# cve-mohd/flow-sim

Measured on AMD Instinct MI355X. Metric: reach-timesteps/sec (batched Preissmann Newton step), higher is better.
Workload: dtype f64

## Files before the change

flow-sim_amd/csrc/fs_abi.hip:

```cpp
#include <hip/hip_runtime.h>

#include <algorithm>
#include <cmath>
#include <condition_variable>
#include <cstdio>
#include <cstdlib>
#include <cstring>
#include <functional>
#include <limits>
#include <mutex>
#include <string>
#include <thread>
#include <vector>

#include "fs_buffer.hpp"
#include "fs_entries.hpp"
#include "fs_host_pack.hpp"

#include <rocprofiler-sdk-roctx/roctx.h>
namespace {
struct TraceRange {
  explicit TraceRange(const char *name) { roctxRangePushA(name); }
  ~TraceRange() { roctxRangePop(); }
};
// ... 163 lines not shown
  fs::DeviceBuffer iters, status;
  fs::DeviceBuffer it_done;
  fs::DeviceBuffer ends_dev;
  fs::PinnedBuffer ends_pin;
  fs::DeviceBuffer open_dev;
  fs::PinnedBuffer open_pin;
  fs::DeviceBuffer derived[8];
  fs::DeviceBuffer dbg;
  Staging stage;
  fs::DeviceBuffer kc_scratch;
  int passes = 0;
  fs::DeviceBuffer team_mail;
  fs::DeviceBuffer team_sync;
  int team_size = 0;
  uint32_t team_epoch = 0;
};

namespace {

template <typename F> auto with_real(const fs_batch *b, F &&f) { return b->d.dtype == FS_F64 ? f(double()) : f(float()); }

dim3 grid_256(size_t n) { return dim3((unsigned)((n + 255) / 256)); }

int upload_to(fs_batch *b, void *dst, const double *src, size_t n) {
  TraceRange range_("flowsim:upload");
  const bool f64 = b->esz == sizeof(double);
  if (f64 || n * b->esz < kStageMin || b->stage.init() != 0) {
    if (f64) {
      HIP_TRY(hipMemcpyAsync(dst, src, n * sizeof(double), hipMemcpyHostToDevice, b->stream));
      HIP_TRY(hipStreamSynchronize(b->stream));
// ... 120 lines not shown
  a.geo_reach_stride = (int64_t)b->geo_reach_stride; a.poly_reach_stride = (int64_t)b->poly_reach_stride;
  a.reach_nodes = b->reach_nodes.get<int32_t>(); a.reach_scheme = b->reach_scheme.get<R>();
  a.reach_kinds = (b->kinds_per_reach[0] || b->kinds_per_reach[1]) ? b->reach_kinds.get<int32_t>() : nullptr;
  fs::BCDesc<R> *bc[2] = {&a.us, &a.ds};
  for (int s = 0; s < 2; ++s) {
    bc[s]->kind = b->bc_kind[s]; bc[s]->stride = b->bc_stride[s];
    bc[s]->params = b->bc_params[s].get<R>(); bc[s]->target = b->bc_target[s].get<R>(); bc[s]->tgt = R(0);
  }
  a.Yprev = b->Yprev.get<R>(); a.stage_hist = b->stage_hist.get<R>(); a.trace = b->trace.get<R>(); a.hydro = b->hydro.get<R>();
  a.iters = b->iters.get<int32_t>(); a.status = b->status.get<int32_t>();
  a.hist_h = b->hist_h.get<R>(); a.hist_Q = b->hist_Q.get<R>();
  a.dbg = b->dbg.get<unsigned long long>();
  a.kc_scratch = b->kc_scratch.get<R>(); a.passes = b->passes;
  a.team_size = b->team_size; a.team_mail = b->team_mail.get<R>(); a.team_sync = b->team_sync.get<unsigned long long>(); a.team_epoch = b->team_epoch;
  a.iter_budget = 0; a.it_done = b->it_done.get<int32_t>();
}

int launch_steps(fs_batch *b, int n_steps, int iter_budget) {
  TraceRange range_(iter_budget > 0 ? "flowsim:iterate" : "flowsim:step");
  std::string why;
  const int hetero = (b->reach_nodes ? 1 : 0) | ((b->reach_scheme || b->kinds_per_reach[0] || b->kinds_per_reach[1]) ? 2 : 0);
  fs::Query q;
  q.dtype = b->d.dtype; q.sec = b->d.section_mode; q.N = b->d.n_nodes; q.usk = b->bc_kind[0]; q.dsk = b->bc_kind[1];
  q.need_diag = (b->d.flags & (FS_FLAG_HISTORY | FS_FLAG_TRACE | FS_FLAG_MONITOR)) != 0; q.need_any = iter_budget > 0; q.hetero = hetero;
  const int chosen = fs::pick(kEntries, kNumEntries, q, fs::overrides_from_environment(), &why);
  const Entry *k = chosen < 0 ? nullptr : &kEntries[chosen];
  if (!k && why.rfind("FS_KERNEL_INDEX", 0) == 0) return fail("fs_batch_step: " + why);
  if (!k && (b->bc_kind[0] == FS_BC_STORAGE_CURVE || b->bc_kind[1] == FS_BC_STORAGE_CURVE))
    return fail("fs_batch_step: FS_BC_STORAGE_CURVE needs section mode FS_SEC_TABLE or FS_SEC_IRREGULAR");
  if (!k) return fail("fs_batch_step: no kernel instantiation for this boundary kind at this size");
  b->kern = k;
  b->passes = 0;
  if (k->key.longk) {
    const size_t chunk = (size_t)64 * k->key.W * k->key.M;
    b->passes = (int)((b->d.n_nodes + chunk - 1) / chunk);
    const bool recompute = b->d.section_mode == FS_SEC_RECT_UNIFORM || b->d.section_mode == FS_SEC_TRAP_UNIFORM;
    const size_t need = recompute ? 0 : (size_t)b->d.n_reaches * 4 * b->passes * chunk;
    HIP_TRY(b->kc_scratch.reserve(need * b->esz));
  }
  b->team_size = 0;
  if (k->key.team) {
    const size_t chunk = (size_t)64 * k->key.W * k->key.M, B = b->d.n_reaches;
    b->team_size = (int)((b->d.n_nodes + chunk - 1) / chunk);
    const size_t need = B * 2 * ((size_t)b->team_size * k->key.W + 1) * fs::kTeamWords * 2;
    bool grew = false;
    HIP_TRY(b->team_mail.reserve(need * sizeof(double), &grew));
    if (grew) HIP_TRY(hipMemsetAsync(b->team_mail.get(), 0, need * sizeof(double), b->stream));
    ++b->team_epoch;
    HIP_TRY(b->team_sync.ensure(sizeof(unsigned long long)));
    HIP_TRY(hipMemsetAsync(b->team_sync.get(), 0, sizeof(unsigned long long), b->stream));
  }
  HIP_TRY(hipEventRecord(b->ev0, b->stream));
  with_real(b, [&](auto real) {
    fs::KernelArgs<decltype(real)> a; fill_args(b, n_steps, a);
    a.iter_budget = iter_budget;
    b->kern->fn(&a, b->d.n_reaches, b->stream);
  });
  HIP_TRY(hipGetLastError());
  HIP_TRY(hipEventRecord(b->ev1, b->stream));
  b->timed = true; b->launches = 1;
  return 0;
}


int check_side(const char *entry, int32_t side) {
  if (side != FS_UPSTREAM && side != FS_DOWNSTREAM) return fail(std::string(entry) + ": side must be FS_UPSTREAM or FS_DOWNSTREAM");
// ... 32 lines not shown

int fill_side_kinds(fs_batch *b, int side, int kind) {
  const size_t B = b->d.n_reaches;
  const std::vector<int32_t> same(B, kind);
  HIP_TRY(hipMemcpy(b->reach_kinds.get<int32_t>() + (size_t)side * B, same.data(), B * 4, hipMemcpyHostToDevice));
  return 0;
}

int begin_at_level0(fs_batch *b) {
  const size_t B = b->d.n_reaches, L = b->d.max_levels;
  HIP_TRY(hipMemsetAsync(b->status.get(), 0, B * 4, b->stream));
  HIP_TRY(hipMemsetAsync(b->iters.get(), 0, L * B * 4, b->stream));
  HIP_TRY(hipMemsetAsync(b->Yprev.get(), 0, B * b->esz, b->stream));
  if (b->trace) HIP_TRY(hipMemsetAsync(b->trace.get(), 0, L * FS_TRACE_CAP * B * b->esz, b->stream));
  HIP_TRY(hipMemsetAsync(b->it_done.get(), 0, B * 4, b->stream));
  b->level = 0; b->iterating = false; b->restart_level = 0;
  b->have_state = true;
  return 0;
}

int init_batch(fs_batch *b) {
  HIP_TRY(hipSetDevice(b->d.device));
  HIP_TRY(hipStreamCreateWithFlags(&b->stream, hipStreamNonBlocking));
  HIP_TRY(hipEventCreate(&b->ev0));
  HIP_TRY(hipEventCreate(&b->ev1));
  const size_t B = b->d.n_reaches, N = b->d.n_nodes, L = b->d.max_levels, esz = b->esz;
  auto zeroed = [&](fs::DeviceBuffer &buf, size_t bytes) -> int {
    HIP_TRY(buf.ensure(bytes));
    HIP_TRY(hipMemsetAsync(buf.get(), 0, bytes, b->stream));
    return 0;
  };
  for (fs::DeviceBuffer *p : {&b->hk, &b->Qk, &b->hg, &b->Qg}) HIP_TRY(p->ensure(B * N * esz));
  if (zeroed(b->hydro, L * 4 * B * esz) || zeroed(b->iters, L * B * 4) || zeroed(b->status, B * 4) || zeroed(b->Yprev, B * esz) ||
      zeroed(b->stage_hist, L * B * esz) || zeroed(b->it_done, B * 4)) return -1;
  if ((b->d.flags & FS_FLAG_TRACE) && zeroed(b->trace, L * FS_TRACE_CAP * B * esz)) return -1;
  if (b->d.flags & FS_FLAG_HISTORY) {
    HIP_TRY(b->hist_h.ensure(L * B * N * esz));
    HIP_TRY(b->hist_Q.ensure(L * B * N * esz));
  }
#ifdef FS_STAMP
  if (zeroed(b->dbg, B * 16 * 12 * 8)) return -1;
#endif
  HIP_TRY(hipStreamSynchronize(b->stream));
  if (B * N * esz >= kStageMin) (void)b->stage.init();
  return 0;
}

}

extern "C" {

int fs_abi_version(void) { return FS_ABI_VERSION; }

int fs_device_count(void) {
  int n = 0;
  if (hipGetDeviceCount(&n) != hipSuccess) return 0;
// ... 546 lines not shown

double fs_batch_last_step_ms(fs_batch *b) {
  if (!b || !b->timed) return -1.0;
  float ms = 0.f;
  if (hipEventSynchronize(b->ev1) != hipSuccess) return -1.0;
  if (hipEventElapsedTime(&ms, b->ev0, b->ev1) != hipSuccess) return -1.0;
  return (double)ms;
}

int32_t fs_batch_last_launch_count(fs_batch *b) { return b ? b->launches : 0; }

#ifdef FS_STAMP
int fs_debug_stamps(fs_batch *b, unsigned long long *out) {
  if (!b || !out || !b->dbg) return fail("fs_debug_stamps: not available");
  HIP_TRY(hipStreamSynchronize(b->stream));
  HIP_TRY(hipMemcpy(out, b->dbg.get(), (size_t)b->d.n_reaches * 16 * 12 * 8, hipMemcpyDeviceToHost));
  return 0;
}
#endif

int32_t fs_kernel_table_size(void) { return kNumEntries; }

int fs_kernel_table_entry(int32_t i, int32_t *out) {
  if (i < 0 || i >= kNumEntries || !out) return fail("fs_kernel_table_entry: index out of range");
  const fs::KernelKey &e = kEntries[i].key;
  out[0] = e.dtype; out[1] = e.sec; out[2] = e.M; out[3] = e.W; out[4] = e.full; out[5] = e.bck; out[6] = e.diag; out[7] = e.longk;
  return 0;
}

int32_t fs_batch_kernel_index(fs_batch *b) { return (b && b->kern) ? (int32_t)(b->kern - kEntries) : -1; }

int32_t fs_kernel_table_entry_tail(int32_t i) { return (i >= 0 && i < kNumEntries) ? kEntries[i].key.tail : -2; }
int32_t fs_kernel_table_entry_team(int32_t i) { return (i >= 0 && i < kNumEntries) ? kEntries[i].key.team : -2; }

int32_t fs_batch_poly_tables(fs_batch *b) { return (b && b->poly_x) ? (b->poly_K > 0 ? 1 : 0) : -1; }

int fs_batch_kernel_info(fs_batch *b, int32_t *cells_per_thread, int32_t *waves_per_reach, int32_t *lds_bytes,
                         int32_t *vgprs) {
  if (!b) return fail("null handle");
  hipFuncAttributes at;
  HIP_TRY(hipFuncGetAttributes(&at, b->kern->kp));
  if (cells_per_thread) *cells_per_thread = b->kern->key.M;
  if (waves_per_reach) *waves_per_reach = b->kern->key.W;
  if (lds_bytes) *lds_bytes = (int32_t)at.sharedSizeBytes;
  if (vgprs) *vgprs = at.numRegs;
// ... 5 lines not shown
```

flow-sim_amd/csrc/fs_dispatch.hpp:

```cpp
#pragma once
#include <algorithm>
#include <cstdio>
#include <cstdlib>
#include <string>
#include <tuple>

#include "../../include/flowsim_abi.h"
#include "fs_entry_list.hpp"

#ifndef FS_ST_HD
#ifdef __HIPCC__
#define FS_ST_HD __host__ __device__
#else
#define FS_ST_HD
#endif
#endif

namespace fs {

FS_ST_HD constexpr bool bc_is_light(int kind) { return kind != FS_BC_RATING_POWER && kind < FS_BC_STORAGE_CURVE; }

struct KernelKey {
  int dtype;
  int sec;
  int M;
  int W;
  int full;
  int bck;
  int diag;
  int longk;
  int tail;
  int team;
};
#define FS_KEY(KIND, R, DT, SEC, M, W, FULL, BCK, DIAG, TAIL) \
  fs::KernelKey{DT, SEC, M, W, FULL, (int)(BCK), DIAG, FS_KIND_##KIND == FS_KIND_LONG, TAIL, FS_KIND_##KIND == FS_KIND_TEAM}
// ... 3 lines not shown
  int N;
  int usk, dsk;
  bool need_diag = false;
  bool need_any = false;
  int hetero = 0;
};

struct Overrides {
  bool force_index = false;
  int index = 0;
  std::string index_text;
  int M = 0, W = 0;
  bool general_only = false;
  bool no_team = false;
  int team_M = -1;
};

inline Overrides overrides_from_environment() {
  Overrides o;
  if (const char *env = std::getenv("FS_KERNEL_INDEX")) { o.force_index = true; o.index = std::atoi(env); o.index_text = env; }
  if (const char *env = std::getenv("FS_KERNEL_SHAPE")) std::sscanf(env, "%d,%d", &o.M, &o.W);
  if (const char *env = std::getenv("FS_KERNEL_GENERAL")) o.general_only = env[0] == '1';
  o.no_team = std::getenv("FS_NO_TEAM") != nullptr;
  if (const char *env = std::getenv("FS_TEAM_M")) o.team_M = std::max(std::atoi(env), 0);
  return o;
}

inline bool fits(const KernelKey &k, const Query &q, const Overrides &o) {
  if (k.dtype != q.dtype || k.sec != q.sec) return false;
  const long grid = 64L * k.W * k.M, cap = grid * ((k.longk || k.team) ? 64 / k.W : 1);
  if (q.N > cap || q.N > 32768) return false;
  if (k.full && (k.team ? q.N % grid != 0 : q.N != cap)) return false;
  if (k.tail >= 0 && (q.N - 1) % k.M != k.tail) return false;
  if (k.team && (q.N <= 4096 || q.N <= grid || o.no_team || (o.team_M >= 0 && o.team_M != k.M))) return false;
  if ((q.hetero & 1) && (k.full || k.tail >= 0)) return false;
  if ((q.hetero & 2) && k.bck > 0) return false;
  if (q.need_diag && !k.diag) return false;
  if (q.need_any && k.bck != -1) return false;
// ... 34 lines not shown
```

flow-sim_amd/csrc/fs_kernel.hpp:

```cpp
#pragma once
#include <type_traits>
#include "fs_device.hpp"
#include "fs_poly.hpp"

namespace fs {

#ifdef FS_STAMP
#define FS_T(i)                                                         \
  do {                                                                  \
    const unsigned long long now_ = __builtin_amdgcn_s_memtime();       \
    stamp_[i] += now_ - tprev_;                                         \
    tprev_ = now_;                                                      \
  } while (0)
#else
#define FS_T(i) do { } while (0)
#endif

template <typename R> __host__ __device__ constexpr R finite_max() { return sizeof(R) == 8 ? R(1.7976931348623157e308) : R(3.4028234e38); }
template <typename R> __host__ __device__ constexpr R eps_of() { return sizeof(R) == 8 ? R(2.220446049250313e-16) : R(1.1920929e-7); }

__device__ __forceinline__ int hi_abs(double v) { return __double2hiint(v) & 0x7fffffff; }
__device__ __forceinline__ int hi_abs(float v) { return __float_as_int(v) & 0x7fffffff; }
template <typename R> __host__ __device__ constexpr int growth_limit_bits() { return sizeof(R) == 8 ? ((1023 + 10) << 20) : ((127 + 10) << 23); }
__device__ __forceinline__ int max_(int a, int b) { return a > b ? a : b; }
// ... 21 lines not shown
  R *trace;
  unsigned long long *dbg;
  int64_t geo_reach_stride;
  int64_t poly_reach_stride;
  const int32_t *reach_nodes;
  const R *reach_scheme;
  const int32_t *reach_kinds;
  const R *poly_tz;
  int32_t poly_K;
  R *kc_scratch;
  int32_t passes;
  int32_t team_size;
  R *team_mail;
  unsigned long long *team_sync;
  uint32_t team_epoch;
};
constexpr int kTeamSlots = 64;
constexpr unsigned long long kTeamPatience = 16000000000ull;
constexpr int kTeamWords = 12;

template <typename R, int SEC> struct Geometry;

constexpr int kTeamSleep = 1;
typedef unsigned int fs_u4 __attribute__((ext_vector_type(4)));
constexpr int kTeamAuxSc1 = 16;
__device__ __forceinline__ void team_put2(__amdgpu_buffer_rsrc_t r, unsigned off, unsigned long long bits, unsigned long long tag) {
  fs_u4 v;
  v.x = (unsigned)bits; v.y = (unsigned)(bits >> 32); v.z = (unsigned)tag; v.w = (unsigned)(tag >> 32);
  __builtin_amdgcn_raw_buffer_store_b128(v, r, off, 0, kTeamAuxSc1);
}
// ... 16 lines not shown
    n = a.geo_uniform[(size_t)FS_RU_MANNING * a.B + reach];
    z_us = a.geo_uniform[(size_t)FS_RU_Z_US * a.B + reach];
    z_ds = a.geo_uniform[(size_t)FS_RU_Z_DS * a.B + reach];
    rb = R(1) / b; rn = R(1) / n;
    inv_nm1 = R(1) / R(n_nodes - 1);
    dz = (z_ds - z_us) * inv_nm1;
  }
  __device__ __forceinline__ R bed_step(int) const { return dz; }
  __device__ __forceinline__ R terms_T() const { return b; }
  __device__ __forceinline__ R rT_const() const { return rb; }
  __device__ __forceinline__ R bed(int node) const {
    const R w2 = R(node) * inv_nm1;
    return z_us * (R(1) - w2) + z_ds * w2;
  }
  __device__ __forceinline__ NodeTerms<R> terms(int, R h, R Q) const { return node_terms_rect(b, rb, n, h, Q); }
  __device__ __forceinline__ SecParams<R> section(int node) const {
    SecParams<R> s;
    s.z = bed(node); s.b = b; s.m = R(0); s.nm = n; s.nl = n; s.nr = n; s.hbf = R(0);
    s.bl = R(0); s.br = R(0); s.mfp = R(0); s.curv = R(0); s.compound = false;
    s.sm = R(1); s.rnm = rn; s.sfp = R(1); s.Tb = b; s.Am = R(0); s.Pm = b; s.km15 = s.kl15 = s.kr15 = R(0);
    return s;
  }
  template <int BCK, int SIDE>
  __device__ __forceinline__ BCRow<R> boundary(const BCDesc<R> &bc, int reach, int B, int level, int node, R h, R Q,
                                               R Qold, R dt, R Yprev, R *Ynew, int *flag) const {
    if (BCK == 1 || (BCK >= 2 && bc_is_light(BCK - 2)))
      return bc_eval_rect(pinned<BCK, SIDE>(bc), (LdsParams<R>)bc.params, level, b, n, node == 0 ? z_us : z_ds, h, Q, Qold, dt, Yprev, Ynew, flag);
    return bc_eval<BCK != 0>(pinned<BCK, SIDE>(bc), reach, B, level, section(node), h, Q, Qold, dt, Yprev, Ynew, flag);
  }
};
// ... 203 lines not shown
}

template <typename R, int SEC, int M, int W, bool RAGGED = true, int BCK = 0, bool DIAG = true, int TAIL = -1, bool TEAM = false>
__global__ __launch_bounds__(64 * W, (min_waves<R, SEC, M, W, BCK, TEAM>())) void preissmann_step_kernel(const KernelArgs<R> a) {
  static_assert(M >= 2, "a lane's segment needs two rows (its up and its down row)");
  constexpr bool kTail = TAIL >= 0;
  constexpr bool kTeam = TEAM;
  static_assert(!kTeam || (W > 1 && BCK >= 0 && !kTail), "team form: multi-wave kernels, boundary kinds of the device");
  static_assert(!kTail || (RAGGED && W == 1 && TAIL < M && SEC == FS_SEC_TABLE && BCK >= 2), "tail-only form: ragged one-wave table kernels compiled for a boundary pair");
  constexpr int T = 64 * W;
  using Geo = Geometry<R, SEC>;
  constexpr int kSaveTermsMaxMF64 = 2;
  constexpr bool kSaveTerms = !Geometry<R, SEC>::kConstT && (M <= 2 || (sizeof(R) == 8 && M <= kSaveTermsMaxMF64));
  constexpr bool kRegGeo = SEC == FS_SEC_TABLE && W == 1 && M <= 2;
  constexpr bool kFlatBC = BCK >= 2 && sizeof(R) == 8 && SEC == FS_SEC_TRAP_UNIFORM;
  __shared__ Smem<R, M, W, kSaveTerms, kTeam> sm;

  const int t = threadIdx.x, lane = t & 63, wave = t >> 6;
  int job = blockIdx.x;
  if constexpr (kTeam) {
    if (t == 0) sm.xjob = (int)__hip_atomic_fetch_add(a.team_sync, 1ull, __ATOMIC_RELAXED, __HIP_MEMORY_SCOPE_AGENT);
    __syncthreads();
    job = sm.xjob;
  }
  const int G = kTeam ? a.team_size : 1;
  const int reach = kTeam ? job / G : job, member = kTeam ? job - reach * G : 0;
  const int gt = member * T + t;
  auto mbox = [&](int par) __attribute__((always_inline)) {
    const size_t bytes = (size_t)(G * W + 1) * kTeamWords * 16;
    char *base = reinterpret_cast<char *>(a.team_mail) + ((size_t)reach * 2 + par) * bytes;
// ... 63 lines not shown
  auto last_node_terms = [&](const NodeTerms<R> &first) __attribute__((always_inline)) {
    auto rol = [](R v) { return dpp_mov<0x134>(v); };
    NodeTerms<R> r;
    r.A = rol(first.A); r.T = rol(first.T); r.Se = rol(first.Se); r.eAT = rol(first.eAT); r.eQ = rol(first.eQ); r.v = rol(first.v);
    r.rT = rol(first.rT);
    return r;
  };
  auto write_level_constants = [&](const R(&hh)[M + 1], const R(&QQ)[M + 1]) __attribute__((always_inline)) {
    NodeTerms<R> L = terms_at(0, hh[0], QQ[0]);
    NodeTerms<R> Rlast;
    if (kShareNode) Rlast = last_node_terms(L);
#pragma unroll
    for (int c = 0; c < M; ++c) {
      const NodeTerms<R> Rn = (kShareNode && c == M - 1) ? Rlast : terms_at(c + 1, hh[c + 1], QQ[c + 1]);
      const R sumA = L.A + Rn.A;
      sm.kc[0][c][t] = fma_(cqk, QQ[c + 1] - QQ[c], -(sumA * r2dt));
      sm.kc[1][c][t] = fma_(cqk, fma_(QQ[c + 1], Rn.v, -(QQ[c] * L.v)), -((QQ[c + 1] + QQ[c]) * r2dt));
      sm.kc[2][c][t] = ghthk * sumA;
      sm.kc[3][c][t] = fma_(cqk, geo.bed_step(s0 + c) + (hh[c + 1] - hh[c]), hthk * (L.Se + Rn.Se));
      L = Rn;
    }
  };
  auto save_terms = [&](int j, const NodeTerms<R> &nt) __attribute__((always_inline)) {
    if constexpr (kSaveTerms) { sm.nt[0][j][t] = nt.A; sm.nt[1][j][t] = nt.Se; sm.nt[2][j][t] = nt.v; }
  };
  auto level_constants_from_saved = [&](const R(&hh)[M + 1], const R(&QQ)[M + 1]) __attribute__((always_inline)) {
    if constexpr (kSaveTerms) {
      R A0 = sm.nt[0][0][t], Se0 = sm.nt[1][0][t], v0 = sm.nt[2][0][t];
#pragma unroll
      for (int c = 0; c < M; ++c) {
        const R A1 = sm.nt[0][c + 1][t], Se1 = sm.nt[1][c + 1][t], v1 = sm.nt[2][c + 1][t];
        const R sumA = A0 + A1;
        sm.kc[0][c][t] = fma_(cqk, QQ[c + 1] - QQ[c], -(sumA * r2dt));
        sm.kc[1][c][t] = fma_(cqk, fma_(QQ[c + 1], v1, -(QQ[c] * v0)), -((QQ[c + 1] + QQ[c]) * r2dt));
        sm.kc[2][c][t] = ghthk * sumA;
// ... 33 lines not shown
    __syncthreads();
    if (pinned<BCK, 1>(dsd).kind == FS_BC_NORMAL_DEPTH && geo.hint_init(N - 1) != -2 && sm.bcp[1][1] == geo.bed(N - 1)) {
      fuseD = true;
      const R S0 = sm.bcp[1][0];
      fuse_sg = S0 < R(0) ? R(-1) : R(1); fuse_rt = sqrt_(fabs_(S0));
    }
  }
  const bool ds_storage = BCK >= 2 ? bc_is_storage(BCK - 2) : bc_is_storage(dsd.kind);
  R Yprev = (ds_storage && gt == tD) ? a.Yprev[reach] : R(0);
  int status = a.status[reach];
  constexpr bool kMonitor = DIAG;
  bool warn = status == FS_ILL_CONDITIONED;
  if (warn) status = FS_OK;
  int parity = 0;
  int exchanges = 0;
  if (t == 0) { sm.xflag[0] = 0; sm.xflag[1] = 0; }
  __syncthreads();

  {
    R hk[M + 1], Qk[M + 1];
#pragma unroll
    for (int j = 0; j <= M; ++j) {
      const int node = min(s0 + j, N - 1);
      hk[j] = a.hk[base + node]; Qk[j] = a.Qk[base + node];
    }
    if (gt == tD) {
#pragma unroll
      for (int j = RAGGED ? 0 : M - 1; j < M; ++j) if (j == jD) QoldD = Qk[j];
    }
    write_level_constants(hk, Qk);
  }
#ifdef FS_STAMP
  unsigned long long stamp_[12] = {0, 0, 0, 0, 0, 0, 0, 0, 0, 0, 0, 0};
  unsigned long long tprev_ = __builtin_amdgcn_s_memtime();
#endif
  for (int step = 0; step < a.n_steps && status == FS_OK; ++step) {
    const int level = a.level0 + step + 1;
    if (usd.target) usd.tgt = usd.target[(size_t)level * a.B + reach];
    if (dsd.target) dsd.tgt = dsd.target[(size_t)level * a.B + reach];
    int it = kBudget ? it_entry : 0;
    int budget = (kBudget && a.iter_budget > 0) ? a.iter_budget : 0x7fffffff;
    bool converged = false;
    R Ynew = Yprev;
    while (!converged && status == FS_OK) {
      R dh[M + 1], dQ[M + 1];
      if (kBudget && budget-- <= 0) break;
      ++it;
      if constexpr (BCK <= 0) { if (it - 1 >= max_iter_of()) { status = FS_MAX_ITER; break; } }
      else
      if (it - 1 >= a.max_iter) { status = FS_MAX_ITER; break; }
      parity ^= 1;
      bool grow = false;
      FS_T(7);

      int kco = t;
      asm volatile("" : "+v"(kco));
      int ln = lane;
      asm volatile("" : "+v"(ln));
      const R *kcb = &sm.kc[0][0][0] + kco;
      int kco2 = kco + 2 * M * T;
      if constexpr (4 * M * T * sizeof(R) > 65536) asm volatile("" : "+v"(kco2));
      const R *kcb2 = &sm.kc[0][0][0] + kco2;

      BCRow<R> Urow, Drow;
      Drow.dh = R(1); Drow.dq = R(0); Drow.res = R(0);
      R nrm2 = R(0);
      int myflag = 0;
      if constexpr (kFlatBC) {
        R dummy = R(0), YnewAll = Yprev;
        int fU = 0, fD = 0;
        Urow = geo.template boundary<BCK, 0>(usd, reach, a.B, level, 0, h[0], Q[0], R(0), dt, R(0), &dummy, &fU);
        R hD = h[0], QD = Q[0];
#pragma unroll
        for (int j = RAGGED ? 1 : M - 1; j < M; ++j) if (j == jD) { hD = h[j]; QD = Q[j]; }
        Drow = geo.template boundary<BCK, 1>(dsd, reach, a.B, level, N - 1, hD, QD, QoldD, dt, Yprev, &YnewAll, &fD);
        const bool isD = gt == tD;
// ... 41 lines not shown
          if constexpr (kTeam) {
            const unsigned o = (unsigned)(G * W) * kTeamWords * 16u;
            const unsigned long long tg = ((unsigned long long)a.team_epoch << 32) | (unsigned)(exchanges + 1);
            const __amdgpu_buffer_rsrc_t mb = mbox(parity);
            team_put2(mb, o, __double_as_longlong((double)(x + y)), tg); team_put2(mb, o + 16, __double_as_longlong((double)(x - y)), tg);
            team_put2(mb, o + 32, __double_as_longlong((double)(-Urow.res)), tg);
          } else if constexpr (kW1Lanes) {
            xb0 = x + y; xb1 = x - y; xb2 = -Urow.res;
          } else {
          sm.xbc[parity][0] = x + y; sm.xbc[parity][1] = x - y; sm.xbc[parity][2] = -Urow.res;
          }
        }
        R rcPrev = R(0);
#pragma unroll
        for (int c = 0; c < M; ++c) {
          const R k0 = kcb[(0 * M + c) * T], k1 = kcb[(1 * M + c) * T], k2 = kcb2[(0 * M + c) * T], k3 = kcb2[(1 * M + c) * T];
          const NodeTerms<R> Rn = (kShareNode && c == M - 1) ? Rlast : terms_at(c + 1, h[c + 1], Q[c + 1]);
          save_terms(c + 1, Rn);
          const R i2tR = dt * Rn.rT;
          if (!Geo::kConstT) iTn[c + 1] = i2tR;
          Row<R> row;
          {
            const R sumA = L.A + Rn.A;
            const R Cres = sumA * r2dt + cq * (Q[c + 1] - Q[c]) + k0;
            const R gA = fma_(ghth, sumA, k2);
            const R S = cq * (geo.bed_step(s0 + c) + (h[c + 1] - h[c])) + hth * (L.Se + Rn.Se) + k3;
            const R Mres = (Q[c + 1] + Q[c]) * r2dt + cq * (Q[c + 1] * Rn.v - Q[c] * L.v) + k1 + gA * S;
            const R gAdt = gA * dt, gAx = gA * hx, sdt = ghdt * S;
            const R X0 = fma_(gAdt, fma_(hth, L.eAT, -(cq * L.rT)), fma_(dtcq, L.v * L.v, sdt));
            const R X1 = fma_(gAdt, fma_(hth, Rn.eAT, cq * Rn.rT), fma_(-dtcq, Rn.v * Rn.v, sdt));
            const R Y0 = fma_(gAx, L.eQ, kap - L.v);
// ... 35 lines not shown
          if (c == 0) {
            seg.d1 = row.al; seg.d2 = row.D; seg.d3 = row.de; seg.rd = row.rho0;
          } else {
            const R r = frcp(seg.d2);
            const R R1 = seg.d1 * r, R2 = seg.d3 * r, R3 = seg.rd * r;
            LocalElim<R> &e = el[c - 1];
            e.R1.put(R1); e.R2.put(R2); e.R3.put(R3);
            if (!Geo::kConstT) e.qc.put(rcPrev);
            const R rho = fma_(-row.al, rcPrev, row.rho0);
            seg.d1 = row.al * R1; seg.d2 = fma_(row.al, R2, row.D); seg.d3 = row.de; seg.rd = fma_(row.al, R3, rho);
            seg.u1 = fma_(-seg.u3, R1, seg.u1); seg.ru = fma_(-seg.u3, R3, seg.ru); seg.u3 = -(seg.u3 * R2);
          }
          rcPrev = row.rc;
          if constexpr (M >= 8 && sizeof(R) == 4)
            asm volatile("" :: "v"(seg.u1), "v"(seg.u3), "v"(seg.ru), "v"(seg.d1), "v"(seg.d2), "v"(seg.d3), "v"(seg.rd), "v"(rcPrev));
          L = Rn; i2tL = i2tR;
          __builtin_amdgcn_sched_barrier(0);
        }
        seg.rc = rcPrev; rcLast = rcPrev;
        upU1 = seg.u1; upU3 = seg.u3; upRu = seg.ru;
      }
      int gi = 0;
      if constexpr (kMonitor) gi = hi_abs(seg.u3);

      FS_T(0);
      Elim<R> rec[1];
      auto up_level = [&](auto lc) __attribute__((always_inline)) {
        constexpr int l = decltype(lc)::value;
        constexpr int d = 1 << l;
        const Seg<R> left = seg_from_below<d>(seg);
// ... 255 lines not shown
        if constexpr (BCK <= 0) below = err < tol_of(); else
        below = err < a.tol;
        if (DIAG && a.trace && gt == 0 && it <= FS_TRACE_CAP) a.trace[((size_t)level * FS_TRACE_CAP + (it - 1)) * a.B + reach] = err;
      } else {
        if constexpr (BCK <= 0) {
          const R tl = tol_of();
          const R t2 = tl * tl, band = R(16) * eps_of<R>() * t2;
          below = tot < t2 - band ? true : (tot > t2 + band ? false : sqrt_(tot) < tl);
        } else {
        const R t2 = a.tol * a.tol, band = R(16) * eps_of<R>() * t2;
        below = tot < t2 - band ? true : (tot > t2 + band ? false : sqrt_(tot) < a.tol);
        }
      }
      converged = status == FS_OK && below;
      if (converged && grow) warn = true;

      FS_T(5);
      auto load_rec = [&](auto lc) __attribute__((always_inline)) {
        constexpr int l = decltype(lc)::value;
        Elim<R> e;
        const int slot = (64 - (64 >> l)) + (ln >> (l + 1));
        const R *p = &sm.tree[wave][0][slot];
        e.A1 = p[0 * 64]; e.A2 = p[1 * 64]; e.A3 = p[2 * 64]; e.rc = p[3 * 64];
        return e;
      };
      auto down_level = [&](auto lc, const Elim<R> &e) __attribute__((always_inline)) {
        constexpr int l = decltype(lc)::value;
        const R sep = separator(e, pL, mR);
        const bool upper = ((lane >> l) & 1) != 0;
        pL = upper ? e.rc - sep : pL;
// ... 20 lines not shown
        down_level(I2{}, r2);
        const Elim<R> r0 = load_rec(I0{});
        asm volatile("" ::: "memory");
        down_level(I1{}, r1);
        down_level(I0{}, r0);
        asm volatile("" : "+v"(pL), "+v"(mR));
        __builtin_amdgcn_sched_barrier(0);
      }
      R mA = fma_(-upU1, pL, fma_(-upU3, mR, upRu));
      if (W > 1 && lane == 0) mA = mAw;
      R mB = dpp_mov<0x134>(mA);
      if (lane == 63) mB = mBw;

      if (Geo::kConstT) {
        asm volatile("" : "+v"(kco));
        kcb = &sm.kc[0][0][0] + kco;
#pragma unroll
        for (int j = 0; j <= M; ++j) asm volatile("" : "+v"(h[j]), "+v"(Q[j]));
      }
      {
        const R i2tc = dt * geo.rT_const();
        auto i2t_of = [&](int j) { return Geo::kConstT ? i2tc : iTn[j]; };
        auto rc_of = [&](int j) __attribute__((always_inline)) {
          if (Geo::kConstT) {
            const R v = -(geo.terms_T() * (h[j] + h[j + 1]) * r2dt + cq * (Q[j + 1] - Q[j]) + kcb[(0 * M + j) * T]);
            return (RAGGED && s0 + j >= NC) ? R(0) : v;
          }
          return j + 1 < M ? el[j].qc.get() : rcLast;
        };
        R mj = mR;
        {
// ... 40 lines not shown
        FS_T(8);
        if (gt == tD) {
#pragma unroll
          for (int j = RAGGED ? 0 : M - 1; j < M; ++j)
            if (j == jD) {
              a.hydro[((size_t)level * 4 + 2) * a.B + reach] = h[j];
              a.hydro[((size_t)level * 4 + 3) * a.B + reach] = Q[j];
              QoldD = Q[j];
            }
          Yprev = Ynew;
          if (ds_storage) a.stage_hist[(size_t)level * a.B + reach] = Ynew;
        }
        FS_T(9);
        if (kSaveTerms) {
          level_constants_from_saved(h, Q);
        } else {
          write_level_constants(h, Q);
        }
        FS_T(10);
      }

      FS_T(5);
#pragma unroll
      for (int j = 0; j <= M; ++j) { h[j] += dh[j]; Q[j] += dQ[j]; }
    }
    if (status != FS_OK && gt == 0) a.iters[(size_t)level * a.B + reach] = it - (status == FS_MAX_ITER ? 1 : 0);
    if (kBudget && a.iter_budget > 0) {
      if (t == 0) a.it_done[reach] = (converged || status != FS_OK) ? -1 : it;
      if (!converged) break;
    }
  }

#pragma unroll
  for (int j = 0; j < M; ++j)
    if (!RAGGED || s0 + j < N) { hg_p[j] = h[j]; Qg_p[j] = Q[j]; }
  if (gt == 0) a.status[reach] = (status == FS_OK && warn) ? (int)FS_ILL_CONDITIONED : status;
  if (ds_storage && gt == tD) a.Yprev[reach] = Yprev;
#ifdef FS_STAMP
  if (a.dbg && lane == 0)
    for (int i = 0; i < 12; ++i) a.dbg[((size_t)reach * 16 + (member * W + wave) % 16) * 12 + i] = stamp_[i];
#endif
}


template <typename R> struct DeriveArgs {
  int32_t B, N, first, n, section_mode;
  const R *hist_h, *hist_Q;
  const R *geo_uniform, *geo_table;
  const R *poly_x, *poly_z;
  const int32_t *poly_n;
  int64_t geo_reach_stride, poly_reach_stride;
  R *level, *area, *top, *froude, *vel, *cel, *amp, *peak;
  const int32_t *reach_nodes;
};

// ... 110 lines not shown
```

flow-sim_amd/flowsim_amd/_abi.py:

```python
import ctypes as C
import os

_HERE = os.path.dirname(os.path.abspath(__file__))
LIB_PATH = os.path.join(_HERE, "..", "csrc", "libflowsim_hip.so")

F64, F32 = 0, 1
SEC_RECT_UNIFORM, SEC_TRAP_UNIFORM, SEC_TABLE, SEC_IRREGULAR = 0, 1, 2, 3
RU_WIDTH, RU_MANNING, RU_Z_US, RU_Z_DS, RU_NPARAM = 0, 1, 2, 3, 4
TU_SIDE_SLOPE, TU_NPARAM = 4, 5
BC_MAX_PARAMS = 10
GEO_ROWS = ("z_bed", "b_main", "m_main", "n_main", "n_left", "n_right", "is_compound", "h_bf",
            "b_fp_l", "b_fp_r", "m_fp", "curvature")
GEO_NPARAM = len(GEO_ROWS)
(BC_FLOW_HYDROGRAPH, BC_STAGE_HYDROGRAPH, BC_FIXED_DEPTH, BC_NORMAL_DEPTH, BC_RATING_POWER,
 BC_RATING_POLY, BC_RATING_BLEND, BC_STORAGE, BC_STORAGE_CURVE, BC_HOST_ROW) = range(10)
SC_NAMES = ("min_stage", "Y_min", "Y_max", "bed_level", "surface_area", "alpha", "beta", "n_curve", "rc_type", "rc_a",
            "rc_b", "rc_c", "rc_shift", "capture_losses", "reservoir_length", "K_q")
UPSTREAM, DOWNSTREAM = 0, 1
OK, MAX_ITER, NAN, STORAGE_RANGE, ILL_CONDITIONED, TEAM_STALL = 0, 1, 2, 3, 4, 5
FLAG_HISTORY, FLAG_TRACE, FLAG_MONITOR = 1, 2, 4
TRACE_CAP = 64
DERIVE_ALL = 255
ABI_VERSION = 3

# ... 43 lines not shown
    "fs_batch_get_history": (C.c_int, [_P, C.c_int32, C.c_int32, _D, _D]),
    "fs_batch_get_residual_trace": (C.c_int, [_P, C.c_int32, C.c_int32, _D]),
    "fs_batch_get_storage_stage": (C.c_int, [_P, _D]),
    "fs_batch_get_storage_stages": (C.c_int, [_P, C.c_int32, C.c_int32, _D]),
    "fs_batch_derive": (C.c_int, [_P, C.c_int32, C.c_int32, _D, _D, _D, _D, _D, _D, _D, _D]),
    "fs_batch_derive_device": (C.c_int, [_P, C.c_int32, C.c_int32, C.c_int32]),
    "fs_batch_derived_device_ptr": (_P, [_P, C.c_int32]),
    "fs_batch_hydrograph_device_ptr": (_P, [_P]),
    "fs_batch_stream": (_P, [_P]),
    "fs_batch_last_step_ms": (C.c_double, [_P]),
    "fs_batch_last_launch_count": (C.c_int32, [_P]),
    "fs_batch_kernel_info": (C.c_int, [_P, _I, _I, _I, _I]),
    "fs_kernel_table_size": (C.c_int32, []),
    "fs_kernel_table_entry": (C.c_int, [C.c_int32, _I]),
    "fs_batch_kernel_index": (C.c_int32, [_P]),
    "fs_batch_poly_tables": (C.c_int32, [_P]),
    "fs_kernel_table_entry_tail": (C.c_int32, [C.c_int32]),
    "fs_kernel_table_entry_team": (C.c_int32, [C.c_int32]),
}

_lib = None


class FlowsimError(RuntimeError):
    pass


def lib():
    global _lib
    if _lib is None:
# ... 40 lines not shown
```

flow-sim_amd/flowsim_amd/batch.py:

```python
from __future__ import annotations

import ctypes as C
from dataclasses import dataclass, field
from typing import Optional, Sequence

import numpy as np

from . import _abi as A

_KIND_PARAMS = {
    A.BC_FLOW_HYDROGRAPH: (), A.BC_STAGE_HYDROGRAPH: ("bed_level",), A.BC_FIXED_DEPTH: ("initial_depth",),
    A.BC_NORMAL_DEPTH: ("bed_slope", "bed_level"), A.BC_RATING_POWER: ("a", "b", "stage_shift", "bed_level"),
    A.BC_RATING_POLY: ("a", "b", "c", "stage_shift", "bed_level"),
    A.BC_RATING_BLEND: ("stage0", "buffer", "lo0", "lo1", "lo2", "hi0", "hi1", "hi2", "dY", "bed_level"),
    A.BC_STORAGE: ("surface_area", "min_stage", "Y_min", "Y_max", "bed_level"),
}


@dataclass
class BoundarySpec:
    kind: int
    params: dict = field(default_factory=dict)
    target: Optional[np.ndarray] = None

# ... 283 lines not shown

    def last_step_ms(self):
        return self._lib.fs_batch_last_step_ms(self._h)

    def kernel_info(self):
        v = [C.c_int32() for _ in range(4)]
        A.check(self._lib.fs_batch_kernel_info(self._h, *[C.byref(x) for x in v]), "kernel_info")
        return dict(cells_per_thread=v[0].value, waves_per_reach=v[1].value, lds_bytes=v[2].value, vgprs=v[3].value)

    def poly_tables(self):
        return self._lib.fs_batch_poly_tables(self._h)

    def kernel_index(self):
        return self._lib.fs_batch_kernel_index(self._h)

    def derive_device(self, first=0, n=None, fields=A.DERIVE_ALL):
        n = self.level + 1 - first if n is None else n
        A.check(self._lib.fs_batch_derive_device(self._h, first, n, int(fields)), "derive_device")
        names = self.DERIVED + ("peak_amplitude",)
        return {k: self._lib.fs_batch_derived_device_ptr(self._h, i) for i, k in enumerate(names) if fields & (1 << i)}

    def hydrograph_device_ptr(self):
        return self._lib.fs_batch_hydrograph_device_ptr(self._h)
```

include/flowsim_abi.h:

```cpp
#ifndef FLOWSIM_ABI_H
#define FLOWSIM_ABI_H

#include <stdint.h>

#ifdef __cplusplus
extern "C" {
#endif

#define FS_ABI_VERSION 3

typedef struct fs_batch fs_batch;

enum { FS_F64 = 0, FS_F32 = 1 };

enum { FS_SEC_RECT_UNIFORM = 0, FS_SEC_TRAP_UNIFORM = 1, FS_SEC_TABLE = 2, FS_SEC_IRREGULAR = 3 };

enum { FS_RU_WIDTH = 0, FS_RU_MANNING = 1, FS_RU_Z_US = 2, FS_RU_Z_DS = 3, FS_RU_NPARAM = 4 };
enum { FS_TU_SIDE_SLOPE = 4, FS_TU_NPARAM = 5 };

enum {
  FS_GEO_Z_BED = 0, FS_GEO_B_MAIN, FS_GEO_M_MAIN, FS_GEO_N_MAIN, FS_GEO_N_LEFT, FS_GEO_N_RIGHT,
  FS_GEO_IS_COMPOUND, FS_GEO_H_BANKFULL, FS_GEO_B_FP_LEFT, FS_GEO_B_FP_RIGHT, FS_GEO_M_FP,
  FS_GEO_CURVATURE, FS_GEO_NPARAM
};
// ... 104 lines not shown
enum { FS_DERIVE_LEVEL = 1, FS_DERIVE_AREA = 2, FS_DERIVE_TOP_WIDTH = 4, FS_DERIVE_FROUDE = 8, FS_DERIVE_VELOCITY = 16,
       FS_DERIVE_CELERITY = 32, FS_DERIVE_AMPLITUDE = 64, FS_DERIVE_PEAK_AMPLITUDE = 128, FS_DERIVE_ALL = 255 };
int fs_batch_derive_device(fs_batch *b, int32_t first_level, int32_t n_levels, int32_t fields);
void *fs_batch_derived_device_ptr(fs_batch *b, int32_t field_index);

void *fs_batch_hydrograph_device_ptr(fs_batch *b);
void *fs_batch_stream(fs_batch *b);

double fs_batch_last_step_ms(fs_batch *b);
int32_t fs_batch_last_launch_count(fs_batch *b);
int fs_batch_kernel_info(fs_batch *b, int32_t *cells_per_thread, int32_t *waves_per_reach,
                         int32_t *lds_bytes, int32_t *vgprs);
int32_t fs_kernel_table_size(void);
int fs_kernel_table_entry(int32_t i, int32_t *out);
int32_t fs_batch_kernel_index(fs_batch *b);
int32_t fs_kernel_table_entry_tail(int32_t i);
int32_t fs_kernel_table_entry_team(int32_t i);
int32_t fs_batch_poly_tables(fs_batch *b);

#ifdef __cplusplus
}
#endif
#endif
```

Measured before the change: 11.76 million.

## Park last Newton iterate's level constants in global memory and reload on convergence

For f64 rectangular uniform multi-wave kernels, the final Newton iteration writes the momentum and continuity level-constant pairs (kc0/kc1 packed as 2-wide vectors) to a per-reach global park buffer. When that iteration converges, the pairs are copied back into LDS asynchronously with global_load_lds, and only the cheap area-dependent remainder is recomputed. This avoids the full write_level_constants recomputation at the timestep boundary. The cost is extra global stores on every speculative iteration, vmcnt waits, a reordered LDS layout, plus stats counters and an env opt-out.

```diff
diff --git a/flow-sim_amd/csrc/fs_abi.hip b/flow-sim_amd/csrc/fs_abi.hip
--- a/flow-sim_amd/csrc/fs_abi.hip
+++ b/flow-sim_amd/csrc/fs_abi.hip
@@ -201,6 +201,10 @@
   fs::DeviceBuffer team_sync;
   int team_size = 0;
   uint32_t team_epoch = 0;
+  fs::DeviceBuffer park;
+  bool park_refused = false;
+  bool park_live = false;
+  fs::DeviceBuffer park_stats;
 };
 
 namespace {
@@ -351,6 +355,7 @@
   a.kc_scratch = b->kc_scratch.get<R>(); a.passes = b->passes;
   a.team_size = b->team_size; a.team_mail = b->team_mail.get<R>(); a.team_sync = b->team_sync.get<unsigned long long>(); a.team_epoch = b->team_epoch;
   a.iter_budget = 0; a.it_done = b->it_done.get<int32_t>();
+  a.park = b->park_live ? b->park.get<R>() : nullptr; a.park_stats = b->park_stats.get<int32_t>();
 }
 
 int launch_steps(fs_batch *b, int n_steps, int iter_budget) {
@@ -360,7 +365,8 @@
   fs::Query q;
   q.dtype = b->d.dtype; q.sec = b->d.section_mode; q.N = b->d.n_nodes; q.usk = b->bc_kind[0]; q.dsk = b->bc_kind[1];
   q.need_diag = (b->d.flags & (FS_FLAG_HISTORY | FS_FLAG_TRACE | FS_FLAG_MONITOR)) != 0; q.need_any = iter_budget > 0; q.hetero = hetero;
-  const int chosen = fs::pick(kEntries, kNumEntries, q, fs::overrides_from_environment(), &why);
+  const fs::Overrides env = fs::overrides_from_environment();
+  const int chosen = fs::pick(kEntries, kNumEntries, q, env, &why);
   const Entry *k = chosen < 0 ? nullptr : &kEntries[chosen];
   if (!k && why.rfind("FS_KERNEL_INDEX", 0) == 0) return fail("fs_batch_step: " + why);
   if (!k && (b->bc_kind[0] == FS_BC_STORAGE_CURVE || b->bc_kind[1] == FS_BC_STORAGE_CURVE))
@@ -387,6 +393,23 @@
     HIP_TRY(b->team_sync.ensure(sizeof(unsigned long long)));
     HIP_TRY(hipMemsetAsync(b->team_sync.get(), 0, sizeof(unsigned long long), b->stream));
   }
+  b->park_live = false;
+  if (fs::level_park_class(k->key.dtype == FS_F64, k->key.sec, k->key.M, k->key.W, k->key.full != 0, k->key.bck, k->key.diag != 0, k->key.team != 0) &&
+      !k->key.longk && k->key.tail < 0) {
+    const size_t B = b->d.n_reaches, need = B * k->key.M * 64 * k->key.W * 2 * b->esz;
+    if (!env.no_level_park && !b->park_refused) {
+      if (b->park.reserve(need) == hipSuccess) {
+        b->park_live = true;
+      } else {
+        (void)hipGetLastError();
+        b->park.reset(); b->park_refused = true;
+      }
+    }
+    if (!b->park_stats) {
+      HIP_TRY(b->park_stats.ensure(3 * B * 4));
+      HIP_TRY(hipMemsetAsync(b->park_stats.get(), 0, 3 * B * 4, b->stream));
+    }
+  }
   HIP_TRY(hipEventRecord(b->ev0, b->stream));
   with_real(b, [&](auto real) {
     fs::KernelArgs<decltype(real)> a; fill_args(b, n_steps, a);
@@ -449,6 +472,7 @@
   HIP_TRY(hipMemsetAsync(b->Yprev.get(), 0, B * b->esz, b->stream));
   if (b->trace) HIP_TRY(hipMemsetAsync(b->trace.get(), 0, L * FS_TRACE_CAP * B * b->esz, b->stream));
   HIP_TRY(hipMemsetAsync(b->it_done.get(), 0, B * 4, b->stream));
+  if (b->park_stats) HIP_TRY(hipMemsetAsync(b->park_stats.get(), 0, 3 * B * 4, b->stream));
   b->level = 0; b->iterating = false; b->restart_level = 0;
   b->have_state = true;
   return 0;
@@ -474,7 +498,7 @@
     HIP_TRY(b->hist_Q.ensure(L * B * N * esz));
   }
 #ifdef FS_STAMP
-  if (zeroed(b->dbg, B * 16 * 12 * 8)) return -1;
+  if (zeroed(b->dbg, B * 16 * fs::kStampPhases * 8)) return -1;
 #endif
   HIP_TRY(hipStreamSynchronize(b->stream));
   if (B * N * esz >= kStageMin) (void)b->stage.init();
@@ -1051,7 +1075,13 @@
 int fs_debug_stamps(fs_batch *b, unsigned long long *out) {
   if (!b || !out || !b->dbg) return fail("fs_debug_stamps: not available");
   HIP_TRY(hipStreamSynchronize(b->stream));
-  HIP_TRY(hipMemcpy(out, b->dbg.get(), (size_t)b->d.n_reaches * 16 * 12 * 8, hipMemcpyDeviceToHost));
+  HIP_TRY(hipMemcpy2D(out, 12 * 8, b->dbg.get(), fs::kStampPhases * 8, 12 * 8, (size_t)b->d.n_reaches * 16, hipMemcpyDeviceToHost));
+  return 0;
+}
+int fs_debug_stamps_all(fs_batch *b, unsigned long long *out) {
+  if (!b || !out || !b->dbg) return fail("fs_debug_stamps_all: not available");
+  HIP_TRY(hipStreamSynchronize(b->stream));
+  HIP_TRY(hipMemcpy(out, b->dbg.get(), (size_t)b->d.n_reaches * 16 * fs::kStampPhases * 8, hipMemcpyDeviceToHost));
   return 0;
 }
 #endif
@@ -1066,6 +1096,20 @@
 }
 
 int32_t fs_batch_kernel_index(fs_batch *b) { return (b && b->kern) ? (int32_t)(b->kern - kEntries) : -1; }
+
+int fs_batch_level_pass_stats(fs_batch *b, int64_t *out) {
+  if (!b || !out) return fail("fs_batch_level_pass_stats: null argument");
+  out[0] = out[1] = out[2] = 0;
+  if (!b->park_stats) return 0;
+  FS_ON_DEVICE(b);
+  HIP_TRY(hipStreamSynchronize(b->stream));
+  const size_t B = b->d.n_reaches;
+  std::vector<int32_t> host(3 * B);
+  HIP_TRY(hipMemcpy(host.data(), b->park_stats.get(), 3 * B * 4, hipMemcpyDeviceToHost));
+  for (int i = 0; i < 3; ++i)
+    for (size_t r = 0; r < B; ++r) out[i] += host[(size_t)i * B + r];
+  return 0;
+}
 
 int32_t fs_kernel_table_entry_tail(int32_t i) { return (i >= 0 && i < kNumEntries) ? kEntries[i].key.tail : -2; }
 int32_t fs_kernel_table_entry_team(int32_t i) { return (i >= 0 && i < kNumEntries) ? kEntries[i].key.team : -2; }
diff --git a/flow-sim_amd/csrc/fs_dispatch.hpp b/flow-sim_amd/csrc/fs_dispatch.hpp
--- a/flow-sim_amd/csrc/fs_dispatch.hpp
+++ b/flow-sim_amd/csrc/fs_dispatch.hpp
@@ -19,6 +19,10 @@
 namespace fs {
 
 FS_ST_HD constexpr bool bc_is_light(int kind) { return kind != FS_BC_RATING_POWER && kind < FS_BC_STORAGE_CURVE; }
+
+FS_ST_HD constexpr bool level_park_class(bool f64, int sec, int M, int W, bool full, int bck, bool diag, bool team) {
+  return f64 && sec == FS_SEC_RECT_UNIFORM && W > 1 && M >= 8 && full && bck >= 2 && !diag && !team;
+}
 
 struct KernelKey {
   int dtype;
@@ -52,6 +56,7 @@
   bool general_only = false;
   bool no_team = false;
   int team_M = -1;
+  bool no_level_park = false;
 };
 
 inline Overrides overrides_from_environment() {
@@ -60,6 +65,7 @@
   if (const char *env = std::getenv("FS_KERNEL_SHAPE")) std::sscanf(env, "%d,%d", &o.M, &o.W);
   if (const char *env = std::getenv("FS_KERNEL_GENERAL")) o.general_only = env[0] == '1';
   o.no_team = std::getenv("FS_NO_TEAM") != nullptr;
+  o.no_level_park = std::getenv("FS_NO_LEVEL_PARK") != nullptr;
   if (const char *env = std::getenv("FS_TEAM_M")) o.team_M = std::max(std::atoi(env), 0);
   return o;
 }
diff --git a/flow-sim_amd/csrc/fs_kernel.hpp b/flow-sim_amd/csrc/fs_kernel.hpp
--- a/flow-sim_amd/csrc/fs_kernel.hpp
+++ b/flow-sim_amd/csrc/fs_kernel.hpp
@@ -5,6 +5,7 @@
 
 namespace fs {
 
+constexpr int kStampPhases = 14;
 #ifdef FS_STAMP
 #define FS_T(i)                                                         \
   do {                                                                  \
@@ -59,6 +60,8 @@
   R *team_mail;
   unsigned long long *team_sync;
   uint32_t team_epoch;
+  R *park;
+  int32_t *park_stats;
 };
 constexpr int kTeamSlots = 64;
 constexpr unsigned long long kTeamPatience = 16000000000ull;
@@ -105,6 +108,7 @@
     return z_us * (R(1) - w2) + z_ds * w2;
   }
   __device__ __forceinline__ NodeTerms<R> terms(int, R h, R Q) const { return node_terms_rect(b, rb, n, h, Q); }
+  __device__ __forceinline__ R area(R h) const { return b * h; }
   __device__ __forceinline__ SecParams<R> section(int node) const {
     SecParams<R> s;
     s.z = bed(node); s.b = b; s.m = R(0); s.nm = n; s.nl = n; s.nr = n; s.hbf = R(0);
@@ -338,6 +342,8 @@
   constexpr bool kSaveTerms = !Geometry<R, SEC>::kConstT && (M <= 2 || (sizeof(R) == 8 && M <= kSaveTermsMaxMF64));
   constexpr bool kRegGeo = SEC == FS_SEC_TABLE && W == 1 && M <= 2;
   constexpr bool kFlatBC = BCK >= 2 && sizeof(R) == 8 && SEC == FS_SEC_TRAP_UNIFORM;
+  constexpr bool kPark = level_park_class(sizeof(R) == 8, SEC, M, W, !RAGGED, BCK, DIAG, TEAM) && Geo::kConstT && !kTail;
+  typedef R fs_pair __attribute__((ext_vector_type(2)));
   __shared__ Smem<R, M, W, kSaveTerms, kTeam> sm;
 
   const int t = threadIdx.x, lane = t & 63, wave = t >> 6;
@@ -431,11 +437,33 @@
     for (int c = 0; c < M; ++c) {
       const NodeTerms<R> Rn = (kShareNode && c == M - 1) ? Rlast : terms_at(c + 1, hh[c + 1], QQ[c + 1]);
       const R sumA = L.A + Rn.A;
+      if constexpr (kPark) {
+        sm.kc[2][c][t] = fma_(cqk, QQ[c + 1] - QQ[c], -(sumA * r2dt));
+        sm.kc[3][c][t] = ghthk * sumA;
+        fs_pair pr;
+        pr.x = fma_(cqk, fma_(QQ[c + 1], Rn.v, -(QQ[c] * L.v)), -((QQ[c + 1] + QQ[c]) * r2dt));
+        pr.y = fma_(cqk, geo.bed_step(s0 + c) + (hh[c + 1] - hh[c]), hthk * (L.Se + Rn.Se));
+        reinterpret_cast<fs_pair *>(&sm.kc[0][0][0])[c * T + t] = pr;
+      } else {
       sm.kc[0][c][t] = fma_(cqk, QQ[c + 1] - QQ[c], -(sumA * r2dt));
       sm.kc[1][c][t] = fma_(cqk, fma_(QQ[c + 1], Rn.v, -(QQ[c] * L.v)), -((QQ[c + 1] + QQ[c]) * r2dt));
       sm.kc[2][c][t] = ghthk * sumA;
       sm.kc[3][c][t] = fma_(cqk, geo.bed_step(s0 + c) + (hh[c + 1] - hh[c]), hthk * (L.Se + Rn.Se));
+      }
       L = Rn;
+    }
+  };
+  auto write_level_remainder = [&](const R(&hh)[M + 1], const R(&QQ)[M + 1]) __attribute__((always_inline)) {
+    if constexpr (kPark) {
+      R A0 = geo.area(hh[0]);
+#pragma unroll
+      for (int c = 0; c < M; ++c) {
+        const R A1 = geo.area(hh[c + 1]);
+        const R sumA = A0 + A1;
+        sm.kc[2][c][t] = fma_(cqk, QQ[c + 1] - QQ[c], -(sumA * r2dt));
+        sm.kc[3][c][t] = ghthk * sumA;
+        A0 = A1;
+      }
     }
   };
   auto save_terms = [&](int j, const NodeTerms<R> &nt) __attribute__((always_inline)) {
@@ -499,6 +527,12 @@
   if (warn) status = FS_OK;
   int parity = 0;
   int exchanges = 0;
+  const bool park_on = kPark && a.park != nullptr;
+  int it_acc = 0;
+  int n_fed = 0, n_miss = 0, n_plain = 0;
+  typedef __attribute__((address_space(1))) fs_pair *GlobalPair;
+  typedef __attribute__((address_space(1))) char *GlobalBytes;
+  const GlobalBytes park_b = kPark ? (GlobalBytes)a.park + (size_t)reach * M * T * sizeof(fs_pair) : nullptr;
   if (t == 0) { sm.xflag[0] = 0; sm.xflag[1] = 0; }
   __syncthreads();
 
@@ -516,7 +550,7 @@
     write_level_constants(hk, Qk);
   }
 #ifdef FS_STAMP
-  unsigned long long stamp_[12] = {0, 0, 0, 0, 0, 0, 0, 0, 0, 0, 0, 0};
+  unsigned long long stamp_[kStampPhases] = {0, 0, 0, 0, 0, 0, 0, 0, 0, 0, 0, 0, 0, 0};
   unsigned long long tprev_ = __builtin_amdgcn_s_memtime();
 #endif
   for (int step = 0; step < a.n_steps && status == FS_OK; ++step) {
@@ -542,9 +576,16 @@
       asm volatile("" : "+v"(kco));
       int ln = lane;
       asm volatile("" : "+v"(ln));
-      const R *kcb = &sm.kc[0][0][0] + kco;
+      const R *kcb = &sm.kc[0][0][0] + (kPark ? 2 * kco : kco);
       int kco2 = kco + 2 * M * T;
       if constexpr (4 * M * T * sizeof(R) > 65536) asm volatile("" : "+v"(kco2));
+      bool park_now = false;
+      if constexpr (kPark) {
+        asm volatile("s_waitcnt vmcnt(0)" ::: "memory");
+        park_now = park_on && it == it_acc;
+      }
+      unsigned pko = (unsigned)t * (unsigned)sizeof(fs_pair);
+      if constexpr (kPark) asm volatile("" : "+v"(pko));
       const R *kcb2 = &sm.kc[0][0][0] + kco2;
 
       BCRow<R> Urow, Drow;
@@ -616,7 +657,13 @@
         R rcPrev = R(0);
 #pragma unroll
         for (int c = 0; c < M; ++c) {
-          const R k0 = kcb[(0 * M + c) * T], k1 = kcb[(1 * M + c) * T], k2 = kcb2[(0 * M + c) * T], k3 = kcb2[(1 * M + c) * T];
+          R k0, k1, k2, k3;
+          if constexpr (kPark) {
+            const fs_pair pr = *reinterpret_cast<const fs_pair *>(kcb + 2 * c * T);
+            k0 = kcb2[(0 * M + c) * T]; k2 = kcb2[(1 * M + c) * T]; k1 = pr.x; k3 = pr.y;
+          } else {
+            k0 = kcb[(0 * M + c) * T]; k1 = kcb[(1 * M + c) * T]; k2 = kcb2[(0 * M + c) * T]; k3 = kcb2[(1 * M + c) * T];
+          }
           const NodeTerms<R> Rn = (kShareNode && c == M - 1) ? Rlast : terms_at(c + 1, h[c + 1], Q[c + 1]);
           save_terms(c + 1, Rn);
           const R i2tR = dt * Rn.rT;
@@ -682,6 +729,15 @@
           rcPrev = row.rc;
           if constexpr (M >= 8 && sizeof(R) == 4)
             asm volatile("" :: "v"(seg.u1), "v"(seg.u3), "v"(seg.ru), "v"(seg.d1), "v"(seg.d2), "v"(seg.d3), "v"(seg.rd), "v"(rcPrev));
+          if constexpr (kPark) {
+            if (park_now) {
+              asm volatile("" :: "v"(seg.u1), "v"(seg.u3), "v"(seg.ru), "v"(seg.d1), "v"(seg.d2), "v"(seg.d3), "v"(seg.rd), "v"(rcPrev));
+              fs_pair pr;
+              pr.x = fma_(cqk, fma_(Q[c + 1], Rn.v, -(Q[c] * L.v)), -((Q[c + 1] + Q[c]) * r2dt));
+              pr.y = fma_(cqk, geo.bed_step(s0 + c) + (h[c + 1] - h[c]), hthk * (L.Se + Rn.Se));
+              *(GlobalPair)(park_b + c * T * sizeof(fs_pair) + pko) = pr;
+            }
+          }
           L = Rn; i2tL = i2tR;
           __builtin_amdgcn_sched_barrier(0);
         }
@@ -967,6 +1023,25 @@
       }
       converged = status == FS_OK && below;
       if (converged && grow) warn = true;
+      bool fed = false;
+      if constexpr (kPark) {
+        fed = park_now && converged;
+        if (park_now && !converged) ++n_miss;
+        if (fed) {
+          asm volatile("s_waitcnt vmcnt(0)" ::: "memory");
+          const int ws = __builtin_amdgcn_readfirstlane(wave);
+          typedef __attribute__((address_space(3))) fs_pair *LdsPair;
+          const LdsPair slot0 = (LdsPair)reinterpret_cast<fs_pair *>(&sm.kc[0][0][0]) + ws * 64;
+#if defined(__HIP_DEVICE_COMPILE__)
+#pragma unroll
+          for (int c = 0; c < M; ++c)
+            __builtin_amdgcn_global_load_lds((GlobalPair)(park_b + c * T * sizeof(fs_pair) + pko), slot0 + c * T, 16, 0, kTeamAuxSc1);
+#else
+          (void)slot0;
+#endif
+          FS_T(12);
+        }
+      }
 
       FS_T(5);
       auto load_rec = [&](auto lc) __attribute__((always_inline)) {
@@ -1017,7 +1092,7 @@
 
       if (Geo::kConstT) {
         asm volatile("" : "+v"(kco));
-        kcb = &sm.kc[0][0][0] + kco;
+        kcb = &sm.kc[0][0][0] + (kPark ? kco + 2 * M * T : kco);
 #pragma unroll
         for (int j = 0; j <= M; ++j) asm volatile("" : "+v"(h[j]), "+v"(Q[j]));
       }
@@ -1088,9 +1163,15 @@
         FS_T(9);
         if (kSaveTerms) {
           level_constants_from_saved(h, Q);
+        } else if (kPark && fed) {
+          write_level_remainder(h, Q);
+          ++n_fed;
+          FS_T(13);
         } else {
           write_level_constants(h, Q);
-        }
+          if constexpr (kPark) ++n_plain;
+        }
+        if constexpr (kPark) it_acc = it;
         FS_T(10);
       }
 
@@ -1105,6 +1186,12 @@
     }
   }
 
+  if constexpr (kPark) {
+    asm volatile("s_waitcnt vmcnt(0)" ::: "memory");
+    if (t == 0 && a.park_stats) {
+      a.park_stats[reach] += n_fed; a.park_stats[(size_t)a.B + reach] += n_miss; a.park_stats[(size_t)2 * a.B + reach] += n_plain;
+    }
+  }
 #pragma unroll
   for (int j = 0; j < M; ++j)
     if (!RAGGED || s0 + j < N) { hg_p[j] = h[j]; Qg_p[j] = Q[j]; }
@@ -1112,7 +1199,7 @@
   if (ds_storage && gt == tD) a.Yprev[reach] = Yprev;
 #ifdef FS_STAMP
   if (a.dbg && lane == 0)
-    for (int i = 0; i < 12; ++i) a.dbg[((size_t)reach * 16 + (member * W + wave) % 16) * 12 + i] = stamp_[i];
+    for (int i = 0; i < kStampPhases; ++i) a.dbg[((size_t)reach * 16 + (member * W + wave) % 16) * kStampPhases + i] = stamp_[i];
 #endif
 }
 
diff --git a/flow-sim_amd/flowsim_amd/_abi.py b/flow-sim_amd/flowsim_amd/_abi.py
--- a/flow-sim_amd/flowsim_amd/_abi.py
+++ b/flow-sim_amd/flowsim_amd/_abi.py
@@ -81,6 +81,7 @@
     "fs_kernel_table_size": (C.c_int32, []),
     "fs_kernel_table_entry": (C.c_int, [C.c_int32, _I]),
     "fs_batch_kernel_index": (C.c_int32, [_P]),
+    "fs_batch_level_pass_stats": (C.c_int, [_P, C.POINTER(C.c_int64)]),
     "fs_batch_poly_tables": (C.c_int32, [_P]),
     "fs_kernel_table_entry_tail": (C.c_int32, [C.c_int32]),
     "fs_kernel_table_entry_team": (C.c_int32, [C.c_int32]),
diff --git a/flow-sim_amd/flowsim_amd/batch.py b/flow-sim_amd/flowsim_amd/batch.py
--- a/flow-sim_amd/flowsim_amd/batch.py
+++ b/flow-sim_amd/flowsim_amd/batch.py
@@ -321,6 +321,11 @@
     def kernel_index(self):
         return self._lib.fs_batch_kernel_index(self._h)
 
+    def level_pass_stats(self):
+        out = (C.c_int64 * 3)()
+        A.check(self._lib.fs_batch_level_pass_stats(self._h, out), "level_pass_stats")
+        return tuple(int(x) for x in out)
+
     def derive_device(self, first=0, n=None, fields=A.DERIVE_ALL):
         n = self.level + 1 - first if n is None else n
         A.check(self._lib.fs_batch_derive_device(self._h, first, n, int(fields)), "derive_device")
diff --git a/include/flowsim_abi.h b/include/flowsim_abi.h
--- a/include/flowsim_abi.h
+++ b/include/flowsim_abi.h
@@ -142,6 +142,7 @@
 int32_t fs_kernel_table_size(void);
 int fs_kernel_table_entry(int32_t i, int32_t *out);
 int32_t fs_batch_kernel_index(fs_batch *b);
+int fs_batch_level_pass_stats(fs_batch *b, int64_t *out);
 int32_t fs_kernel_table_entry_tail(int32_t i);
 int32_t fs_kernel_table_entry_team(int32_t i);
 int32_t fs_batch_poly_tables(fs_batch *b);
```

After: 11.46 million. -2.5%, worse.
